# jameschapman19/cca_zoo

Measured on NVIDIA H100. Metric: rcca_fit_per_s, higher is better.
Workload: dtype tf32x3b+f32

## Files before the change

cca_zoo_b200/csrc/common.cuh:

```cuda
#pragma once

#include <cuda.h>
#include <cuda_runtime.h>
#include <stdint.h>
#include <stdio.h>

namespace ccab {

void set_error(const char* fmt, ...);
int cuda_fail(cudaError_t e, const char* what);

#define CCAB_CUDA(expr)                                              \
  do {                                                               \
    cudaError_t _e = (expr);                                         \
    if (_e != cudaSuccess) return ::ccab::cuda_fail(_e, #expr);      \
  } while (0)

#define CCAB_CHECK_ARG(cond, ...)        \
  do {                                   \
    if (!(cond)) {                       \
      ::ccab::set_error(__VA_ARGS__);    \
      return -1;                         \
    }                                    \
  } while (0)

void count_launches(int n);
long launch_count();

static inline int64_t ceil_div(int64_t a, int64_t b) { return (a + b - 1) / b; }

#ifdef __CUDACC__

__device__ __forceinline__ uint32_t smem_u32(const void* p) {
  return static_cast<uint32_t>(__cvta_generic_to_shared(p));
}

template <int N>
__device__ __forceinline__ void setmaxnreg_dec() { asm volatile("setmaxnreg.dec.sync.aligned.u32 %0;" ::"n"(N)); }
template <int N>
__device__ __forceinline__ void setmaxnreg_inc() { asm volatile("setmaxnreg.inc.sync.aligned.u32 %0;" ::"n"(N)); }

__device__ __forceinline__ void mbar_init(uint64_t* bar, uint32_t count) {
  asm volatile("mbarrier.init.shared::cta.b64 [%0], %1;" ::"r"(smem_u32(bar)), "r"(count) : "memory");
}
__device__ __forceinline__ void fence_mbar_init() {
  asm volatile("fence.mbarrier_init.release.cluster;" ::: "memory");
}
__device__ __forceinline__ void mbar_arrive(uint64_t* bar) {
  asm volatile("mbarrier.arrive.shared::cta.b64 _, [%0];" ::"r"(smem_u32(bar)) : "memory");
}
__device__ __forceinline__ void mbar_arrive_expect_tx(uint64_t* bar, uint32_t bytes) {
  asm volatile("mbarrier.arrive.expect_tx.shared::cta.b64 _, [%0], %1;" ::"r"(smem_u32(bar)), "r"(bytes)
               : "memory");
}
__device__ __forceinline__ bool mbar_try_wait(uint64_t* bar, uint32_t parity) {
  uint32_t ok;
  asm volatile(
      "{\n\t.reg .pred P1;\n\t"
      "mbarrier.try_wait.parity.shared::cta.b64 P1, [%1], %2;\n\t"
      "selp.b32 %0, 1, 0, P1;\n\t}\n"
      : "=r"(ok)
      : "r"(smem_u32(bar)), "r"(parity)
      : "memory");
  return ok != 0;
}
__device__ __forceinline__ void mbar_wait(uint64_t* bar, uint32_t parity) {
  uint32_t spins = 0;
  while (!mbar_try_wait(bar, parity)) {
    if (++spins > (1u << 25)) __trap();
  }
}

__device__ __forceinline__ void tma_load_2d(void* smem_dst, const CUtensorMap* map, uint64_t* bar, int c0, int c1) {
  asm volatile(
      "cp.async.bulk.tensor.2d.shared::cluster.global.mbarrier::complete_tx::bytes [%0], [%1, {%3, %4}], [%2];"
      ::"r"(smem_u32(smem_dst)), "l"(map), "r"(smem_u32(bar)), "r"(c0), "r"(c1)
      : "memory");
}


__device__ __forceinline__ void fence_proxy_async_smem() {
  asm volatile("fence.proxy.async.shared::cta;" ::: "memory");
}
__device__ __forceinline__ void wgmma_fence() { asm volatile("wgmma.fence.sync.aligned;" ::: "memory"); }
__device__ __forceinline__ void wgmma_commit() { asm volatile("wgmma.commit_group.sync.aligned;" ::: "memory"); }
__device__ __forceinline__ void wgmma_wait_all() { asm volatile("wgmma.wait_group.sync.aligned 0;" ::: "memory"); }
__device__ __forceinline__ void wgmma_wait_1() { asm volatile("wgmma.wait_group.sync.aligned 1;" ::: "memory"); }
template <int N>
__device__ __forceinline__ void wgmma_wait() { asm volatile("wgmma.wait_group.sync.aligned %0;" ::"n"(N) : "memory"); }
template <int R>
__device__ __forceinline__ void wgmma_fence_regs(float* d) {
#pragma unroll
  for (int i = 0; i < R; ++i) asm volatile("" : "+f"(d[i])::"memory");
}
template <int R>
__device__ __forceinline__ void wgmma_fence_regs(uint32_t* a) {
#pragma unroll
  for (int i = 0; i < R; ++i) asm volatile("" : "+r"(a[i])::"memory");
}

__device__ __forceinline__ uint64_t wgmma_desc_k128(uint32_t saddr) {
  return (uint64_t)((saddr >> 4) & 0x3FFF) | ((uint64_t)1 << 16) | ((uint64_t)(1024 >> 4) << 32) |
         ((uint64_t)1 << 62);
}

template <int N>
__device__ __forceinline__ void wgmma_tf32(float* d, uint64_t desc_a, uint64_t desc_b);

template <>
__device__ __forceinline__ void wgmma_tf32<64>(float* d, uint64_t desc_a, uint64_t desc_b) {
  asm volatile(
      "{\n\t.reg .pred p;\n\tsetp.ne.b32 p, %34, 0;\n\t"
      "wgmma.mma_async.sync.aligned.m64n64k8.f32.tf32.tf32 "
      "{%0, %1, %2, %3, %4, %5, %6, %7, %8, %9, %10, %11, %12, %13, %14, %15, %16, %17, %18, %19, %20, %21, %22, %23, %24, %25, %26, %27, %28, %29, %30, %31}, %32, %33, p, 1, 1;\n\t}\n"
      : "+f"(d[0]), "+f"(d[1]), "+f"(d[2]), "+f"(d[3]), "+f"(d[4]), "+f"(d[5]), "+f"(d[6]), "+f"(d[7]), "+f"(d[8]), "+f"(d[9]), "+f"(d[10]), "+f"(d[11]), "+f"(d[12]), "+f"(d[13]), "+f"(d[14]), "+f"(d[15]), "+f"(d[16]), "+f"(d[17]), "+f"(d[18]), "+f"(d[19]), "+f"(d[20]), "+f"(d[21]), "+f"(d[22]), "+f"(d[23]), "+f"(d[24]), "+f"(d[25]), "+f"(d[26]), "+f"(d[27]), "+f"(d[28]), "+f"(d[29]), "+f"(d[30]), "+f"(d[31])
      : "l"(desc_a), "l"(desc_b), "r"(1));
}

template <>
__device__ __forceinline__ void wgmma_tf32<128>(float* d, uint64_t desc_a, uint64_t desc_b) {
  asm volatile(
      "{\n\t.reg .pred p;\n\tsetp.ne.b32 p, %66, 0;\n\t"
      "wgmma.mma_async.sync.aligned.m64n128k8.f32.tf32.tf32 "
      "{%0, %1, %2, %3, %4, %5, %6, %7, %8, %9, %10, %11, %12, %13, %14, %15, %16, %17, %18, %19, %20, %21, %22, %23, %24, %25, %26, %27, %28, %29, %30, %31, %32, %33, %34, %35, %36, %37, %38, %39, %40, %41, %42, %43, %44, %45, %46, %47, %48, %49, %50, %51, %52, %53, %54, %55, %56, %57, %58, %59, %60, %61, %62, %63}, %64, %65, p, 1, 1;\n\t}\n"
      : "+f"(d[0]), "+f"(d[1]), "+f"(d[2]), "+f"(d[3]), "+f"(d[4]), "+f"(d[5]), "+f"(d[6]), "+f"(d[7]), "+f"(d[8]), "+f"(d[9]), "+f"(d[10]), "+f"(d[11]), "+f"(d[12]), "+f"(d[13]), "+f"(d[14]), "+f"(d[15]), "+f"(d[16]), "+f"(d[17]), "+f"(d[18]), "+f"(d[19]), "+f"(d[20]), "+f"(d[21]), "+f"(d[22]), "+f"(d[23]), "+f"(d[24]), "+f"(d[25]), "+f"(d[26]), "+f"(d[27]), "+f"(d[28]), "+f"(d[29]), "+f"(d[30]), "+f"(d[31]), "+f"(d[32]), "+f"(d[33]), "+f"(d[34]), "+f"(d[35]), "+f"(d[36]), "+f"(d[37]), "+f"(d[38]), "+f"(d[39]), "+f"(d[40]), "+f"(d[41]), "+f"(d[42]), "+f"(d[43]), "+f"(d[44]), "+f"(d[45]), "+f"(d[46]), "+f"(d[47]), "+f"(d[48]), "+f"(d[49]), "+f"(d[50]), "+f"(d[51]), "+f"(d[52]), "+f"(d[53]), "+f"(d[54]), "+f"(d[55]), "+f"(d[56]), "+f"(d[57]), "+f"(d[58]), "+f"(d[59]), "+f"(d[60]), "+f"(d[61]), "+f"(d[62]), "+f"(d[63])
      : "l"(desc_a), "l"(desc_b), "r"(1));
}

template <int N>
__device__ __forceinline__ void wgmma_tf32_ra(float* d, const uint32_t* a, uint64_t desc_b);

template <>
__device__ __forceinline__ void wgmma_tf32_ra<128>(float* d, const uint32_t* a, uint64_t desc_b) {
  asm volatile(
      "{\n\t.reg .pred p;\n\tsetp.ne.b32 p, %69, 0;\n\t"
      "wgmma.mma_async.sync.aligned.m64n128k8.f32.tf32.tf32 "
      "{%0, %1, %2, %3, %4, %5, %6, %7, %8, %9, %10, %11, %12, %13, %14, %15, %16, %17, %18, %19, %20, %21, %22, %23, %24, %25, %26, %27, %28, %29, %30, %31, %32, %33, %34, %35, %36, %37, %38, %39, %40, %41, %42, %43, %44, %45, %46, %47, %48, %49, %50, %51, %52, %53, %54, %55, %56, %57, %58, %59, %60, %61, %62, %63}, {%64, %65, %66, %67}, %68, p, 1, 1;\n\t}\n"
      : "+f"(d[0]), "+f"(d[1]), "+f"(d[2]), "+f"(d[3]), "+f"(d[4]), "+f"(d[5]), "+f"(d[6]), "+f"(d[7]), "+f"(d[8]), "+f"(d[9]), "+f"(d[10]), "+f"(d[11]), "+f"(d[12]), "+f"(d[13]), "+f"(d[14]), "+f"(d[15]), "+f"(d[16]), "+f"(d[17]), "+f"(d[18]), "+f"(d[19]), "+f"(d[20]), "+f"(d[21]), "+f"(d[22]), "+f"(d[23]), "+f"(d[24]), "+f"(d[25]), "+f"(d[26]), "+f"(d[27]), "+f"(d[28]), "+f"(d[29]), "+f"(d[30]), "+f"(d[31]), "+f"(d[32]), "+f"(d[33]), "+f"(d[34]), "+f"(d[35]), "+f"(d[36]), "+f"(d[37]), "+f"(d[38]), "+f"(d[39]), "+f"(d[40]), "+f"(d[41]), "+f"(d[42]), "+f"(d[43]), "+f"(d[44]), "+f"(d[45]), "+f"(d[46]), "+f"(d[47]), "+f"(d[48]), "+f"(d[49]), "+f"(d[50]), "+f"(d[51]), "+f"(d[52]), "+f"(d[53]), "+f"(d[54]), "+f"(d[55]), "+f"(d[56]), "+f"(d[57]), "+f"(d[58]), "+f"(d[59]), "+f"(d[60]), "+f"(d[61]), "+f"(d[62]), "+f"(d[63])
      : "r"(a[0]), "r"(a[1]), "r"(a[2]), "r"(a[3]), "l"(desc_b), "r"(1));
}

__device__ __forceinline__ float tf32_hi(float v) { return __uint_as_float(__float_as_uint(v) & 0xFFFFE000u); }
__device__ __forceinline__ float tf32_residual(float v) {
  uint32_t l;
  asm("cvt.rna.tf32.f32 %0, %1;" : "=r"(l) : "f"(v - tf32_hi(v)));
  return __uint_as_float(l);
}

__device__ __forceinline__ uint32_t k128_offset(int row, int kg) {
  return (uint32_t)row * 128u + ((uint32_t)(kg ^ (row & 7)) << 4);
}

template <bool KMAJ, int ROWS>
struct TileStager {
  static constexpr int kItems = ROWS * 8 / 256;
  float v[kItems][4];

  __device__ __forceinline__ static int item_row(int i) { return KMAJ ? i >> 3 : i % ROWS; }
  __device__ __forceinline__ static int item_kg(int i) { return KMAJ ? i & 7 : i / ROWS; }

  __device__ __forceinline__ void load(const float* X, int64_t ld, int rows, int ks, bool vec) {
#pragma unroll
    for (int j = 0; j < kItems; ++j) {
      const int i = threadIdx.x + 256 * j;
      const int r = item_row(i), k = 4 * item_kg(i);
      if (KMAJ) {
        const float* src = X + (int64_t)r * ld + k;
        if (vec && r < rows && k + 4 <= ks) {
          const float4 q = __ldg(reinterpret_cast<const float4*>(src));
          v[j][0] = q.x; v[j][1] = q.y; v[j][2] = q.z; v[j][3] = q.w;
        } else {
#pragma unroll
          for (int e = 0; e < 4; ++e) v[j][e] = (r < rows && k + e < ks) ? __ldg(src + e) : 0.f;
        }
      } else {
#pragma unroll
        for (int e = 0; e < 4; ++e) v[j][e] = (r < rows && k + e < ks) ? __ldg(X + (int64_t)(k + e) * ld + r) : 0.f;
      }
    }
  }

  template <bool X3>
  __device__ __forceinline__ void store(uint8_t* hi, uint8_t* lo) const {
#pragma unroll
    for (int j = 0; j < kItems; ++j) {
      const int i = threadIdx.x + 256 * j;
      const uint32_t off = k128_offset(item_row(i), item_kg(i));
      *reinterpret_cast<float4*>(hi + off) =
          make_float4(tf32_hi(v[j][0]), tf32_hi(v[j][1]), tf32_hi(v[j][2]), tf32_hi(v[j][3]));
      if (X3)
        *reinterpret_cast<float4*>(lo + off) = make_float4(tf32_residual(v[j][0]), tf32_residual(v[j][1]),
                                                           tf32_residual(v[j][2]), tf32_residual(v[j][3]));
    }
  }
};

#endif

}
```

cca_zoo_b200/csrc/moments.cu:

```cuda
#include "moments.cuh"

#include <mutex>
#include <type_traits>

namespace ccab {

int make_layout(int n_views, const int64_t* dims, ColumnLayout* L) {
  CCAB_CHECK_ARG(n_views >= 1 && n_views <= kMaxViews, "n_views must be in [1,%d], got %d", kMaxViews,
                 n_views);
  L->n_views = n_views;
  L->coff[0] = 0;
  L->poff[0] = 0;
  int nb = 0;
  for (int v = 0; v < n_views; ++v) {
    CCAB_CHECK_ARG(dims[v] >= 1 && dims[v] <= kMaxBlocks * kBlk, "bad view width %lld", (long long)dims[v]);
    L->dims[v] = (int)dims[v];
    int b = (int)ceil_div(dims[v], kBlk);
    nb += b;
    L->coff[v + 1] = L->coff[v] + (int)dims[v];
    L->poff[v + 1] = L->poff[v] + b * kBlk;
  }
  CCAB_CHECK_ARG(nb <= kMaxBlocks, "total padded width %d exceeds %d", nb * kBlk, kMaxBlocks * kBlk);
  L->nblocks = nb;
  L->D = L->coff[n_views];
  L->Dp = nb * kBlk;
  return 0;
}

static bool g_prof_on = false;
static cudaEvent_t g_prof_e0 = nullptr, g_prof_e1 = nullptr;
static bool g_prof_valid = false;
void moments_profile_enable(int on) {
  g_prof_on = on != 0;
  g_prof_valid = false;
  if (g_prof_on && !g_prof_e0) {
    cudaEventCreate(&g_prof_e0);
    cudaEventCreate(&g_prof_e1);
  }
}
float moments_profile_last_ms() {
  if (!g_prof_valid) return -1.f;
  float ms = -1.f;
  if (cudaEventSynchronize(g_prof_e1) != cudaSuccess) return -1.f;
  if (cudaEventElapsedTime(&ms, g_prof_e0, g_prof_e1) != cudaSuccess) return -1.f;
  return ms;
}

struct WgParams {
  CUtensorMap map[kMaxViews];
  uint8_t blk_view[kMaxBlocks];
  int blk_col0[kMaxBlocks];
  float* partial;
  float* partial_sum;
  int64_t n_rows, rows_per_split;
  int64_t row_base;
  int nblocks, Dp;
};
static_assert(sizeof(WgParams) <= 4096, "kernel parameter space");

constexpr int kWgXpose = 256;
constexpr int kWgThreads = kWgXpose + 256;
constexpr int kWgKC = 32;
constexpr int kWgTile = kBlk * kWgKC * 4;
constexpr int kWgBox = 32 * kWgKC * 4;

__device__ __forceinline__ uint32_t raw_offset(int k, int m) {
  return (uint32_t)(m >> 5) * kWgBox + k128_offset(k, (m & 31) >> 2) + (uint32_t)(m & 3) * 4;
}

template <bool X3>
struct WgCfg {
  static constexpr int kOps = X3 ? 2 : 1;
  static constexpr int kOpStage = kOps * kWgTile;
  static constexpr int kRawStage = 2 * kWgTile;
  static constexpr int kOpStages = X3 ? 2 : 3;
  static constexpr int kRawStages = 5;
  static constexpr int kBarOff = kOpStages * kOpStage + kRawStages * kRawStage;
  static constexpr int kSumOff = kBarOff + 2 * (kOpStages + kRawStages) * 8;
  static constexpr int kSmem = kSumOff + kBlk * 4 + 1024;
};
static_assert(WgCfg<true>::kSmem <= 227 * 1024 && WgCfg<false>::kSmem <= 227 * 1024, "shared memory per block");
static_assert(WgCfg<true>::kRawStages > WgCfg<true>::kOpStages && WgCfg<false>::kRawStages > WgCfg<false>::kOpStages,
              "the refill of a raw stage must not wait on the MMA warps' current slice");

template <bool X3>
__global__ void __launch_bounds__(kWgThreads, 1) moments_wgmma_kernel(const __grid_constant__ WgParams p) {
  using Cfg = WgCfg<X3>;
  constexpr int NO = Cfg::kOpStages, NR = Cfg::kRawStages;
  extern __shared__ uint8_t smem_raw[];
  uint8_t* smem = smem_raw + ((1024u - (smem_u32(smem_raw) & 1023u)) & 1023u);
  uint8_t* ops = smem;
  uint8_t* raw = smem + NO * Cfg::kOpStage;
  uint64_t* raw_full = reinterpret_cast<uint64_t*>(smem + Cfg::kBarOff);
  uint64_t* raw_empty = raw_full + NR;
  uint64_t* op_full = raw_empty + NR;
  uint64_t* op_empty = op_full + NO;

  int t = blockIdx.x, bi = 0, rowlen = p.nblocks;
  while (t >= rowlen) { t -= rowlen; ++bi; --rowlen; }
  const int bj = bi + t;
  const bool diag = bi == bj;
  const int split = blockIdx.y;
  const int64_t r0 = (int64_t)split * p.rows_per_split;
  const int64_t r1 = min(r0 + p.rows_per_split, p.n_rows);
  const int nch = r1 > r0 ? (int)((r1 - r0 + kWgKC - 1) / kWgKC) : 0;

  if (threadIdx.x == 0) {
    for (int s = 0; s < NR; ++s) {
      mbar_init(&raw_full[s], 1);
      mbar_init(&raw_empty[s], kWgXpose + 8);
    }
    for (int s = 0; s < NO; ++s) {
      mbar_init(&op_full[s], kWgXpose);
      mbar_init(&op_empty[s], 8);
    }
    fence_mbar_init();
  }
  __syncthreads();

  if (threadIdx.x < kWgXpose) {
    setmaxnreg_dec<80>();
    const int m = threadIdx.x % kBlk, h = threadIdx.x / kBlk;
    const CUtensorMap* mapA = &p.map[p.blk_view[bi]];
    const CUtensorMap* mapB = &p.map[p.blk_view[bj]];
    const int colA = p.blk_col0[bi], colB = p.blk_col0[bj];
    auto issue = [&](int c) {
      const int s = c % NR;
      const int row = (int)(p.row_base + r0 + (int64_t)c * kWgKC);
      uint8_t* dst = raw + s * Cfg::kRawStage;
      mbar_arrive_expect_tx(&raw_full[s], diag ? kWgTile : 2 * kWgTile);
#pragma unroll
      for (int q = 0; q < kBlk / 32; ++q) {
        tma_load_2d(dst + q * kWgBox, mapA, &raw_full[s], colA + 32 * q, row);
        if (!diag) tma_load_2d(dst + kWgTile + q * kWgBox, mapB, &raw_full[s], colB + 32 * q, row);
      }
    };
    if (threadIdx.x == 0)
      for (int c = 0; c < min(NR, nch); ++c) issue(c);

    float csum = 0.f;
    auto transpose = [&](const uint8_t* src, uint8_t* hi, uint8_t* lo, bool sums) {
#pragma unroll
      for (int j = 0; j < kWgKC / 8; ++j) {
        const int kg = 2 * j + h;
        float v[4];
#pragma unroll
        for (int e = 0; e < 4; ++e)
          v[e] = *reinterpret_cast<const float*>(src + raw_offset(4 * kg + e, m));
        const uint32_t off = k128_offset(m, kg);
        *reinterpret_cast<float4*>(hi + off) = make_float4(tf32_hi(v[0]), tf32_hi(v[1]), tf32_hi(v[2]), tf32_hi(v[3]));
        if (X3)
          *reinterpret_cast<float4*>(lo + off) = make_float4(tf32_residual(v[0]), tf32_residual(v[1]),
                                                             tf32_residual(v[2]), tf32_residual(v[3]));
        if (sums) csum += (v[0] + v[1]) + (v[2] + v[3]);
      }
    };
    for (int c = 0; c < nch; ++c) {
      const int sr = c % NR, so = c % NO;
      mbar_wait(&raw_full[sr], (c / NR) & 1);
      mbar_wait(&op_empty[so], ((c / NO) & 1) ^ 1);
      uint8_t* dst = ops + so * Cfg::kOpStage;
      transpose(raw + sr * Cfg::kRawStage + (diag ? 0 : kWgTile), dst, dst + kWgTile, diag);
      fence_proxy_async_smem();
      mbar_arrive(&raw_empty[sr]);
      mbar_arrive(&op_full[so]);
      const int rf = c + NR - NO + 1;
      if (threadIdx.x == 0 && rf >= NR && rf < nch) {
        mbar_wait(&raw_empty[rf % NR], (rf / NR - 1) & 1);
        issue(rf);
      }
    }
    if (diag) {
      float* odd = reinterpret_cast<float*>(smem + Cfg::kSumOff);
      if (h) odd[m] = csum;
      asm volatile("bar.sync 1, %0;" ::"n"(kWgXpose) : "memory");
      if (!h) p.partial_sum[(size_t)split * p.Dp + bi * kBlk + m] = csum + odd[m];
    }
  } else {
    setmaxnreg_inc<168>();
    const int wg = (threadIdx.x - kWgXpose) >> 7, lane = threadIdx.x & 31, t = lane & 3;
    const int m = wg * 64 + ((threadIdx.x >> 5) & 3) * 16 + (lane >> 2);
    const int kx = t ^ ((t & 1) << 2);
    const bool swap = t & 1;
    const uint32_t o00 = raw_offset(kx, m), o01 = raw_offset(kx ^ 4, m);
    const uint32_t o10 = raw_offset(kx, m + 8), o11 = raw_offset(kx ^ 4, m + 8);
    float acc[64];
#pragma unroll
    for (int i = 0; i < 64; ++i) acc[i] = 0.f;
    wgmma_fence_regs<64>(acc);
    constexpr int KS = kWgKC / 8;
    uint32_t fa[KS][Cfg::kOps][4] = {};
    for (int c = 0; c < nch; ++c) {
      const int sr = c % NR, so = c % NO;
      mbar_wait(&raw_full[sr], (c / NR) & 1);
      const uint8_t* a_src = raw + sr * Cfg::kRawStage;
      const uint32_t b0 = smem_u32(ops + so * Cfg::kOpStage);
#pragma unroll
      for (int kk = 0; kk < KS; ++kk) {
        wgmma_wait<KS - 1>();
        wgmma_fence_regs<Cfg::kOps * 4>(&fa[kk][0][0]);
        if (kk == KS - 1 && c > 0 && lane == 0) mbar_arrive(&op_empty[(c - 1) % NO]);
        const uint8_t* s = a_src + kk * 1024;
        const float v00 = *reinterpret_cast<const float*>(s + o00), v01 = *reinterpret_cast<const float*>(s + o01);
        const float v10 = *reinterpret_cast<const float*>(s + o10), v11 = *reinterpret_cast<const float*>(s + o11);
        const float a[4] = {swap ? v01 : v00, swap ? v11 : v10, swap ? v00 : v01, swap ? v10 : v11};
#pragma unroll
        for (int i = 0; i < 4; ++i) {
          fa[kk][0][i] = __float_as_uint(tf32_hi(a[i]));
          if constexpr (X3) fa[kk][1][i] = __float_as_uint(tf32_residual(a[i]));
        }
        wgmma_fence_regs<Cfg::kOps * 4>(&fa[kk][0][0]);
        if (kk == KS - 1) {
          __syncwarp();
          if (lane == 0) mbar_arrive(&raw_empty[sr]);
        }
        if (kk == 0) mbar_wait(&op_full[so], (c / NO) & 1);
        const uint64_t b_hi = wgmma_desc_k128(b0 + 32 * kk);
        wgmma_fence();
        if constexpr (X3) {
          const uint64_t b_lo = wgmma_desc_k128(b0 + kWgTile + 32 * kk);
          wgmma_tf32_ra<128>(acc, fa[kk][1], b_hi);
          wgmma_tf32_ra<128>(acc, fa[kk][0], b_lo);
        }
        wgmma_tf32_ra<128>(acc, fa[kk][0], b_hi);
        wgmma_commit();
      }
    }
    wgmma_wait_all();
    wgmma_fence_regs<64>(acc);

    const int warp = (threadIdx.x >> 5) & 3;
    float* P = p.partial + (size_t)split * p.Dp * p.Dp;
    const int row0 = bi * kBlk + wg * 64 + warp * 16 + (lane >> 2);
    const int col0 = bj * kBlk + 2 * (lane & 3);
#pragma unroll
    for (int r = 0; r < 64; r += 2) {
      const int row = row0 + 8 * ((r >> 1) & 1), col = col0 + 8 * (r >> 2);
      *reinterpret_cast<float2*>(P + (size_t)row * p.Dp + col) = make_float2(acc[r], acc[r + 1]);
    }
  }
}
struct SimtParams {
  const void* view_ptr[kMaxViews];
  int64_t view_ld[kMaxViews];
  int view_dim[kMaxViews];
  int view_poff[kMaxViews + 1];
  int n_views;
  int64_t n_rows;
  int64_t rows_per_split;
  int nb64, Dp;
  void* partial;
  void* partial_sum;
};

template <typename T>
__global__ void __launch_bounds__(256) moments_simt_kernel(const SimtParams p) {
  constexpr int KC = 16;
  __shared__ T As[KC][64];
  __shared__ T Bs[KC][64];
  int t = blockIdx.x, bi = 0, rowlen = p.nb64;
  while (t >= rowlen) { t -= rowlen; ++bi; --rowlen; }
  const int bj = bi + t;
  const int split = blockIdx.y;
  const int64_t r0 = split * p.rows_per_split;
  const int64_t r1 = min(r0 + p.rows_per_split, p.n_rows);

  auto locate = [&](int pcol0, int& v, int& c0) {
    v = 0;
    while (v + 1 < p.n_views && p.view_poff[v + 1] <= pcol0) ++v;
    c0 = pcol0 - p.view_poff[v];
  };
  int vA, cA, vB, cB;
  locate(bi * 64, vA, cA);
  locate(bj * 64, vB, cB);
  const T* XA = static_cast<const T*>(p.view_ptr[vA]);
  const T* XB = static_cast<const T*>(p.view_ptr[vB]);
  const int64_t ldA = p.view_ld[vA], ldB = p.view_ld[vB];
  const int dA = p.view_dim[vA], dB = p.view_dim[vB];

  const int tx = threadIdx.x & 15, ty = threadIdx.x >> 4;
  T acc[4][4];
#pragma unroll
  for (int i = 0; i < 4; ++i)
#pragma unroll
    for (int j = 0; j < 4; ++j) acc[i][j] = T(0);
  T csum[4] = {T(0), T(0), T(0), T(0)};
  constexpr int kRun = 2048;
  double fold[4][4], fold_sum[4];
#pragma unroll
  for (int i = 0; i < 4; ++i) {
    fold_sum[i] = 0.0;
#pragma unroll
    for (int j = 0; j < 4; ++j) fold[i][j] = 0.0;
  }
  auto fold_run = [&]() {
#pragma unroll
    for (int i = 0; i < 4; ++i) {
      fold_sum[i] += (double)csum[i];
      csum[i] = T(0);
#pragma unroll
      for (int j = 0; j < 4; ++j) {
        fold[i][j] += (double)acc[i][j];
        acc[i][j] = T(0);
      }
    }
  };

  const int lc = threadIdx.x & 63, lr = threadIdx.x >> 6;
  for (int64_t r = r0; r < r1; r += KC) {
    if (r > r0 && (r - r0) % kRun == 0) fold_run();
#pragma unroll
    for (int i = 0; i < KC / 4; ++i) {
      const int kr = lr + 4 * i;
      const int64_t row = r + kr;
      const bool rv = row < r1;
      As[kr][lc] = (rv && cA + lc < dA) ? XA[row * ldA + cA + lc] : T(0);
      Bs[kr][lc] = (rv && cB + lc < dB) ? XB[row * ldB + cB + lc] : T(0);
    }
    __syncthreads();
#pragma unroll
    for (int k = 0; k < KC; ++k) {
      T a[4], b[4];
#pragma unroll
      for (int i = 0; i < 4; ++i) { a[i] = As[k][ty * 4 + i]; b[i] = Bs[k][tx * 4 + i]; }
#pragma unroll
      for (int i = 0; i < 4; ++i)
#pragma unroll
        for (int j = 0; j < 4; ++j) acc[i][j] = fma(a[i], b[j], acc[i][j]);
      if (ty == 0) {
#pragma unroll
        for (int j = 0; j < 4; ++j) csum[j] += b[j];
      }
    }
    __syncthreads();
  }
  fold_run();
  T* P = static_cast<T*>(p.partial) + (size_t)split * p.Dp * p.Dp;
#pragma unroll
  for (int i = 0; i < 4; ++i)
#pragma unroll
    for (int j = 0; j < 4; ++j)
      P[(size_t)(bi * 64 + ty * 4 + i) * p.Dp + bj * 64 + tx * 4 + j] = (T)fold[i][j];
  if (bi == bj && ty == 0) {
    T* S = static_cast<T*>(p.partial_sum) + (size_t)split * p.Dp;
#pragma unroll
    for (int j = 0; j < 4; ++j) S[bi * 64 + tx * 4 + j] = (T)fold_sum[j];
  }
}

__device__ __forceinline__ void dmma_m8n8k4(double& c0, double& c1, double a, double b) {
  asm volatile("mma.sync.aligned.m8n8k4.row.col.f64.f64.f64.f64 {%0, %1}, {%2}, {%3}, {%0, %1};"
               : "+d"(c0), "+d"(c1)
               : "d"(a), "d"(b));
}

__global__ void __launch_bounds__(256) moments_dmma_kernel(const SimtParams p) {
  constexpr int KC = 16;
  constexpr int LDS = 64 + 4;
  __shared__ double As[2][KC][LDS];
  __shared__ double Bs[2][KC][LDS];
  int t = blockIdx.x, bi = 0, rowlen = p.nb64;
  while (t >= rowlen) { t -= rowlen; ++bi; --rowlen; }
  const int bj = bi + t;
  const int split = blockIdx.y;
  const int64_t r0 = split * p.rows_per_split;
  const int64_t r1 = min(r0 + p.rows_per_split, p.n_rows);

  auto locate = [&](int pcol0, int& v, int& c0) {
    v = 0;
    while (v + 1 < p.n_views && p.view_poff[v + 1] <= pcol0) ++v;
    c0 = pcol0 - p.view_poff[v];
  };
  int vA, cA, vB, cB;
  locate(bi * 64, vA, cA);
  locate(bj * 64, vB, cB);
  const double* XA = static_cast<const double*>(p.view_ptr[vA]);
  const double* XB = static_cast<const double*>(p.view_ptr[vB]);
// ... 142 lines not shown
}

struct TcPlan {
  int total_chunks, num_splits, chunks_per_split, ntiles;
  size_t partial_bytes, sum_bytes;
};

TcPlan plan_tc(const ColumnLayout& L, int64_t n_rows, int mode) {
  const bool x3 = mode != 0;
  TcPlan P;
  P.total_chunks = (int)ceil_div(n_rows, kWgKC);
  P.ntiles = L.nblocks * (L.nblocks + 1) / 2;
  int S = (int)ceil_div(4 * sm_count(), P.ntiles);
  int max_splits = 64;
  if (x3) {
    S = std::max<int64_t>(S, ceil_div(n_rows, 2048));
    max_splits = 256;
  }
  const int min_chunks = 8;
  S = (int)std::min<int64_t>(S, std::max<int64_t>(1, P.total_chunks / min_chunks));
  const int64_t slab = (int64_t)L.Dp * L.Dp * (int64_t)sizeof(float);
  max_splits = (int)std::max<int64_t>(1, std::min<int64_t>(max_splits, ((int64_t)2 << 30) / slab));
  S = std::min(S, max_splits);
  S = std::max(1, std::min(S, P.total_chunks));
  P.chunks_per_split = (int)ceil_div(P.total_chunks, S);
  P.num_splits = (int)ceil_div(P.total_chunks, P.chunks_per_split);
  P.partial_bytes = (size_t)P.num_splits * L.Dp * L.Dp * sizeof(float);
  P.sum_bytes = (size_t)P.num_splits * L.Dp * sizeof(float);
  return P;
}

int64_t tc_rows_cap(const ColumnLayout& L, int mode) {
  if (mode == 0) return (int64_t)1 << 31;
  const int64_t slab = (int64_t)L.Dp * L.Dp * (int64_t)sizeof(float);
  const int64_t max_splits = std::max<int64_t>(1, std::min<int64_t>(256, ((int64_t)2 << 30) / slab));
  return max_splits * 2048;
}

inline size_t align256(size_t x) { return (x + 255) & ~size_t(255); }

struct SimtPlan {
  int nb64, ntiles, num_splits;
  int64_t rows_per_split;
};

SimtPlan plan_simt(const ColumnLayout& L, int64_t n_rows) {
  SimtPlan P;
  P.nb64 = L.Dp / 64;
  P.ntiles = P.nb64 * (P.nb64 + 1) / 2;
  int S = 1;
  if (P.ntiles < 2 * sm_count()) S = (2 * sm_count()) / P.ntiles;
  S = (int)std::min<int64_t>(S, std::max<int64_t>(1, n_rows / 64));
  S = std::max(1, std::min(S, 64));
  P.rows_per_split = ceil_div(ceil_div(n_rows, S), 16) * 16;
  P.num_splits = (int)ceil_div(n_rows, P.rows_per_split);
  return P;
}

}

size_t moments_workspace_bytes(int dtype, int precision, const ColumnLayout& L, int64_t n_rows) {
  if (precision == 2 || dtype == 1) {
    SimtPlan P = plan_simt(L, n_rows);
    size_t el = dtype == 1 ? 8 : 4;
    return align256((size_t)P.num_splits * L.Dp * L.Dp * el) + align256((size_t)P.num_splits * L.Dp * el);
  }
  TcPlan P = plan_tc(L, std::min(n_rows, tc_rows_cap(L, precision)), precision);
  return align256(P.partial_bytes) + align256(P.sum_bytes) + 256;
}

namespace {

typedef CUresult (*EncodeTiledFn)(CUtensorMap*, CUtensorMapDataType, cuuint32_t, void*, const cuuint64_t*,
                                  const cuuint64_t*, const cuuint32_t*, const cuuint32_t*, CUtensorMapInterleave,
                                  CUtensorMapSwizzle, CUtensorMapL2promotion, CUtensorMapFloatOOBfill);

EncodeTiledFn encode_fn() {
  static EncodeTiledFn fn = nullptr;
  static std::once_flag once;
  std::call_once(once, [] {
    void* f = nullptr;
    cudaDriverEntryPointQueryResult q;
    if (cudaGetDriverEntryPoint("cuTensorMapEncodeTiled", &f, cudaEnableDefault, &q) == cudaSuccess &&
        q == cudaDriverEntryPointSuccess)
      fn = reinterpret_cast<EncodeTiledFn>(f);
  });
  return fn;
}

int encode_view_map(CUtensorMap* map, const void* ptr, int64_t n_rows, int64_t d, int64_t ld) {
  EncodeTiledFn enc = encode_fn();
  if (!enc) {
    set_error("cuTensorMapEncodeTiled entry point not available (driver too old?)");
    return -2;
  }
  cuuint64_t gdim[2] = {(cuuint64_t)d, (cuuint64_t)n_rows};
  cuuint64_t gstride[1] = {(cuuint64_t)ld * 4};
  cuuint32_t box[2] = {32, (cuuint32_t)kWgKC};
  cuuint32_t estr[2] = {1, 1};
  CUresult r = enc(map, CU_TENSOR_MAP_DATA_TYPE_FLOAT32, 2, const_cast<void*>(ptr), gdim, gstride, box, estr,
                   CU_TENSOR_MAP_INTERLEAVE_NONE, CU_TENSOR_MAP_SWIZZLE_128B, CU_TENSOR_MAP_L2_PROMOTION_L2_256B,
                   CU_TENSOR_MAP_FLOAT_OOB_FILL_NONE);
  if (r != CUDA_SUCCESS) {
    set_error("cuTensorMapEncodeTiled failed with CUresult %d (d=%lld n=%lld ld=%lld)", (int)r, (long long)d,
              (long long)n_rows, (long long)ld);
    return -3;
  }
  return 0;
}

int moments_tf32_pass(const ColumnLayout& L, WgParams& prm, int64_t row_base, int64_t n_rows, int mode,
                      double* moments_out, void* ws, size_t ws_bytes, cudaStream_t stream, int accumulate);

}

int moments_tf32(const ColumnLayout& L, const void* const* views, const int64_t* lds, int64_t n_rows, int mode,
                 double* moments_out, void* ws, size_t ws_bytes, cudaStream_t stream) {
  CCAB_CHECK_ARG(n_rows >= 1 && n_rows < (int64_t)1 << 31, "n_rows out of range");
  for (int v = 0; v < L.n_views; ++v)
    CCAB_CHECK_ARG((reinterpret_cast<uintptr_t>(views[v]) & 15) == 0 && lds[v] % 4 == 0,
                   "TF32 moments need 16-byte aligned views and lds %% 4 == 0 (view %d: ld %lld)", v,
                   (long long)lds[v]);
  {
    int dev = 0;
    CCAB_CUDA(cudaGetDevice(&dev));
    CCAB_CUDA(cudaSetDevice(dev));
  }
  WgParams prm;
  memset(&prm, 0, sizeof(prm));
  for (int v = 0; v < L.n_views; ++v) {
    int rc = encode_view_map(&prm.map[v], views[v], n_rows, L.dims[v], lds[v]);
    if (rc) return rc;
  }
  int b = 0;
  for (int v = 0; v < L.n_views; ++v)
    for (int c = 0; c < L.dims[v]; c += kBlk, ++b) {
      prm.blk_view[b] = (uint8_t)v;
      prm.blk_col0[b] = c;
    }
  const int64_t cap = tc_rows_cap(L, mode);
  if (n_rows <= cap) return moments_tf32_pass(L, prm, 0, n_rows, mode, moments_out, ws, ws_bytes, stream, 0);
  const int64_t npass = ceil_div(n_rows, cap);
  const int64_t per = std::min(cap, ceil_div(ceil_div(n_rows, npass), 2048) * 2048);
  int pass = 0;
  for (int64_t r0 = 0; r0 < n_rows; r0 += per, ++pass) {
    int rc = moments_tf32_pass(L, prm, r0, std::min(per, n_rows - r0), mode, moments_out, ws, ws_bytes, stream,
                               pass > 0);
    if (rc) return rc;
  }
  return 0;
}

namespace {
int moments_tf32_pass(const ColumnLayout& L, WgParams& prm, int64_t row_base, int64_t n_rows, int mode,
                      double* moments_out, void* ws, size_t ws_bytes, cudaStream_t stream, int accumulate) {
  TcPlan P = plan_tc(L, n_rows, mode);
  const size_t need = align256(P.partial_bytes) + align256(P.sum_bytes) + 256;
  CCAB_CHECK_ARG(ws_bytes >= need, "workspace too small: %zu < %zu", ws_bytes, need);
  uint8_t* w = reinterpret_cast<uint8_t*>((reinterpret_cast<uintptr_t>(ws) + 255) & ~uintptr_t(255));
  float* d_partial = reinterpret_cast<float*>(w);
  float* d_partial_sum = reinterpret_cast<float*>(w + align256(P.partial_bytes));

  prm.partial = d_partial;
  prm.partial_sum = d_partial_sum;
  prm.n_rows = n_rows;
  prm.rows_per_split = (int64_t)P.chunks_per_split * kWgKC;
  prm.row_base = row_base;
  prm.nblocks = L.nblocks;
  prm.Dp = L.Dp;
  dim3 grid(P.ntiles, P.num_splits);
  if (g_prof_on) cudaEventRecord(g_prof_e0, stream);
  if (mode != 0) {
    CCAB_CUDA(cudaFuncSetAttribute(moments_wgmma_kernel<true>, cudaFuncAttributeMaxDynamicSharedMemorySize,
                                   WgCfg<true>::kSmem));
    moments_wgmma_kernel<true><<<grid, kWgThreads, WgCfg<true>::kSmem, stream>>>(prm);
  } else {
    CCAB_CUDA(cudaFuncSetAttribute(moments_wgmma_kernel<false>, cudaFuncAttributeMaxDynamicSharedMemorySize,
                                   WgCfg<false>::kSmem));
    moments_wgmma_kernel<false><<<grid, kWgThreads, WgCfg<false>::kSmem, stream>>>(prm);
  }
  count_launches(1);
  CCAB_CUDA(cudaGetLastError());
  if (g_prof_on) {
    cudaEventRecord(g_prof_e1, stream);
    g_prof_valid = true;
  }

  const size_t total = (size_t)L.Dp * L.Dp + L.Dp;
  int rblocks = (int)std::min<size_t>((total + 255) / 256, (size_t)sm_count() * 8);
  reduce_partials_kernel<float><<<rblocks, 256, 0, stream>>>(d_partial, d_partial_sum, P.num_splits, L.Dp, L.Dp,
                                                            kBlk, moments_out, accumulate); count_launches(1);
  CCAB_CUDA(cudaGetLastError());
  return 0;
}
}

template <typename T>
int moments_simt(const ColumnLayout& L, const void* const* views, const int64_t* lds, int64_t n_rows,
                 double* moments_out, void* ws, size_t ws_bytes, cudaStream_t stream) {
  CCAB_CHECK_ARG(n_rows >= 1, "n_rows must be positive");
  SimtPlan P = plan_simt(L, n_rows);
  const size_t pb = align256((size_t)P.num_splits * L.Dp * L.Dp * sizeof(T));
  const size_t sb = align256((size_t)P.num_splits * L.Dp * sizeof(T));
  CCAB_CHECK_ARG(ws_bytes >= pb + sb, "workspace too small: %zu < %zu", ws_bytes, pb + sb);
  uint8_t* w = static_cast<uint8_t*>(ws);
  SimtParams prm;
  memset(&prm, 0, sizeof(prm));
  for (int v = 0; v < L.n_views; ++v) {
    prm.view_ptr[v] = views[v];
    prm.view_ld[v] = lds[v];
    prm.view_dim[v] = L.dims[v];
  }
  for (int v = 0; v <= L.n_views; ++v) prm.view_poff[v] = L.poff[v];
  prm.n_views = L.n_views;
  prm.n_rows = n_rows;
  prm.rows_per_split = P.rows_per_split;
  prm.nb64 = P.nb64;
  prm.Dp = L.Dp;
  prm.partial = w;
  prm.partial_sum = w + pb;
  dim3 grid(P.ntiles, P.num_splits);
  if constexpr (std::is_same<T, double>::value)
    moments_dmma_kernel<<<grid, 256, 0, stream>>>(prm);
  else
    moments_simt_kernel<T><<<grid, 256, 0, stream>>>(prm);
  count_launches(1);
  CCAB_CUDA(cudaGetLastError());
  const size_t total = (size_t)L.Dp * L.Dp + L.Dp;
  int rblocks = (int)std::min<size_t>((total + 255) / 256, (size_t)sm_count() * 8);
  reduce_partials_kernel<T><<<rblocks, 256, 0, stream>>>(static_cast<const T*>(prm.partial),
                                                        static_cast<const T*>(prm.partial_sum), P.num_splits,
                                                        L.Dp, L.Dp, 64, moments_out); count_launches(1);
  CCAB_CUDA(cudaGetLastError());
  return 0;
}

template int moments_simt<float>(const ColumnLayout&, const void* const*, const int64_t*, int64_t, double*, void*,
                                 size_t, cudaStream_t);
template int moments_simt<double>(const ColumnLayout&, const void* const*, const int64_t*, int64_t, double*, void*,
                                  size_t, cudaStream_t);

__global__ void pack_moments_kernel(const double* __restrict__ mom, int nblocks, int Dp, double n_local,
                                    double* __restrict__ packed) {
  const int nt = nblocks * (nblocks + 1) / 2;
  const int t = blockIdx.x;
  if (t < nt) {
    int bi = 0, rem = t, rowlen = nblocks;
    while (rem >= rowlen) { rem -= rowlen; ++bi; --rowlen; }
    const int bj = bi + rem;
    const double* src = mom + (size_t)bi * kBlk * Dp + (size_t)bj * kBlk;
    double* dst = packed + (size_t)t * kBlk * kBlk;
    for (int e = threadIdx.x; e < kBlk * kBlk; e += blockDim.x) dst[e] = src[(size_t)(e / kBlk) * Dp + (e % kBlk)];
  } else {
    double* dst = packed + (size_t)nt * kBlk * kBlk;
    const double* s = mom + (size_t)Dp * Dp;
    for (int e = threadIdx.x; e < Dp; e += blockDim.x) dst[e] = s[e];
    if (threadIdx.x == 0) { dst[Dp] = n_local; dst[Dp + 1] = 0.0; }
  }
}

__global__ void unpack_moments_kernel(const double* __restrict__ packed, int nblocks, int Dp, double* __restrict__ mom) {
  const int nt = nblocks * (nblocks + 1) / 2;
  const int bi = blockIdx.y, bj = blockIdx.x;
  if (bi < nblocks) {
    double* dst = mom + (size_t)bi * kBlk * Dp + (size_t)bj * kBlk;
    if (bj >= bi) {
      const int t = bi * nblocks - bi * (bi - 1) / 2 + (bj - bi);
      const double* src = packed + (size_t)t * kBlk * kBlk;
      for (int e = threadIdx.x; e < kBlk * kBlk; e += blockDim.x) dst[(size_t)(e / kBlk) * Dp + (e % kBlk)] = src[e];
    } else {
      for (int e = threadIdx.x; e < kBlk * kBlk; e += blockDim.x) dst[(size_t)(e / kBlk) * Dp + (e % kBlk)] = 0.0;
    }
  } else if (bj == 0) {
    const double* src = packed + (size_t)nt * kBlk * kBlk;
    double* s = mom + (size_t)Dp * Dp;
    for (int e = threadIdx.x; e < Dp; e += blockDim.x) s[e] = src[e];
  }
}

__device__ __forceinline__ double multimem_ld_reduce_add_f64(const double* mc_addr) {
  double v;
  asm volatile("multimem.ld_reduce.relaxed.sys.global.add.f64 %0, [%1];" : "=d"(v) : "l"(mc_addr) : "memory");
  return v;
}
__device__ __forceinline__ void multimem_st_f64(double* mc_addr, double v) {
  asm volatile("multimem.st.relaxed.sys.global.f64 [%0], %1;" ::"l"(mc_addr), "d"(v) : "memory");
}
__device__ __forceinline__ void st_release_sys_u32(uint32_t* p, uint32_t v) {
  asm volatile("st.release.sys.global.u32 [%0], %1;" ::"l"(p), "r"(v) : "memory");
}
__device__ __forceinline__ uint32_t ld_acquire_sys_u32(const uint32_t* p) {
  uint32_t v;
  asm volatile("ld.acquire.sys.global.u32 %0, [%1];" : "=r"(v) : "l"(p) : "memory");
  return v;
}

struct ExchangeParams {
  double* mom;
  double* sym;
  double* mc;
  uint32_t* const* pads;
  double* n_total_out;
  double n_local;
  long long packed;
  long long chunk;
  int rank, world, nblocks, Dp;
  unsigned epoch;
};

__device__ __forceinline__ const double* packed_src(const ExchangeParams& p, long long e, int nt) {
  const long long blk = e / (kBlk * kBlk);
  if (blk < nt) {
    int bi = 0, rem = (int)blk, rowlen = p.nblocks;
    while (rem >= rowlen) { rem -= rowlen; ++bi; --rowlen; }
    const int bj = bi + rem;
    const int off = (int)(e - blk * (kBlk * kBlk));
    return p.mom + ((size_t)bi * kBlk + off / kBlk) * p.Dp + (size_t)bj * kBlk + (off % kBlk);
  }
  const long long t = e - (long long)nt * kBlk * kBlk;
  return t < p.Dp ? p.mom + (size_t)p.Dp * p.Dp + t : nullptr;
}

__device__ __forceinline__ void exchange_barrier(const ExchangeParams& p, unsigned value) {
  __threadfence_system();
  __syncthreads();
  if ((int)threadIdx.x < p.world)
    st_release_sys_u32(p.pads[threadIdx.x] + (size_t)blockIdx.x * p.world + p.rank, value);
  if ((int)threadIdx.x < p.world) {
    const uint32_t* slot = p.pads[p.rank] + (size_t)blockIdx.x * p.world + threadIdx.x;
    unsigned spins = 0;
    while ((int)(ld_acquire_sys_u32(slot) - value) < 0) {
      if (++spins > (1u << 26)) {
        printf("ccab: exchange barrier timed out (rank %d cta %d peer %d)\n", p.rank, blockIdx.x, threadIdx.x);
// ... 228 lines not shown
```

Measured before the change: 147.0.

## Add X3B mode computing cross terms of 3xTF32 with BF16 wgmma

Adds a third kernel mode in which the hi×lo and lo×hi correction products of the split-precision moment GEMM run as BF16 m64n128k16 wgmma instead of TF32 k8. The hi parts stay TF32. The transpose stage writes BF16-packed hi and residual operands alongside the TF32 hi tile. The aim is to halve the instruction count of the correction terms and use the faster BF16 tensor-core rate. In exchange the correction terms carry less precision, and the change only takes effect when mode 3 is selected.

New measurement: 162.7 (median of 6 runs). +10.7%, better.

```diff
diff --git a/cca_zoo_b200/csrc/common.cuh b/cca_zoo_b200/csrc/common.cuh
--- a/cca_zoo_b200/csrc/common.cuh
+++ b/cca_zoo_b200/csrc/common.cuh
@@ -138,6 +138,25 @@
       "{%0, %1, %2, %3, %4, %5, %6, %7, %8, %9, %10, %11, %12, %13, %14, %15, %16, %17, %18, %19, %20, %21, %22, %23, %24, %25, %26, %27, %28, %29, %30, %31, %32, %33, %34, %35, %36, %37, %38, %39, %40, %41, %42, %43, %44, %45, %46, %47, %48, %49, %50, %51, %52, %53, %54, %55, %56, %57, %58, %59, %60, %61, %62, %63}, {%64, %65, %66, %67}, %68, p, 1, 1;\n\t}\n"
       : "+f"(d[0]), "+f"(d[1]), "+f"(d[2]), "+f"(d[3]), "+f"(d[4]), "+f"(d[5]), "+f"(d[6]), "+f"(d[7]), "+f"(d[8]), "+f"(d[9]), "+f"(d[10]), "+f"(d[11]), "+f"(d[12]), "+f"(d[13]), "+f"(d[14]), "+f"(d[15]), "+f"(d[16]), "+f"(d[17]), "+f"(d[18]), "+f"(d[19]), "+f"(d[20]), "+f"(d[21]), "+f"(d[22]), "+f"(d[23]), "+f"(d[24]), "+f"(d[25]), "+f"(d[26]), "+f"(d[27]), "+f"(d[28]), "+f"(d[29]), "+f"(d[30]), "+f"(d[31]), "+f"(d[32]), "+f"(d[33]), "+f"(d[34]), "+f"(d[35]), "+f"(d[36]), "+f"(d[37]), "+f"(d[38]), "+f"(d[39]), "+f"(d[40]), "+f"(d[41]), "+f"(d[42]), "+f"(d[43]), "+f"(d[44]), "+f"(d[45]), "+f"(d[46]), "+f"(d[47]), "+f"(d[48]), "+f"(d[49]), "+f"(d[50]), "+f"(d[51]), "+f"(d[52]), "+f"(d[53]), "+f"(d[54]), "+f"(d[55]), "+f"(d[56]), "+f"(d[57]), "+f"(d[58]), "+f"(d[59]), "+f"(d[60]), "+f"(d[61]), "+f"(d[62]), "+f"(d[63])
       : "r"(a[0]), "r"(a[1]), "r"(a[2]), "r"(a[3]), "l"(desc_b), "r"(1));
+}
+
+template <int N>
+__device__ __forceinline__ void wgmma_bf16_ra(float* d, const uint32_t* a, uint64_t desc_b);
+
+template <>
+__device__ __forceinline__ void wgmma_bf16_ra<128>(float* d, const uint32_t* a, uint64_t desc_b) {
+  asm volatile(
+      "{\n\t.reg .pred p;\n\tsetp.ne.b32 p, %69, 0;\n\t"
+      "wgmma.mma_async.sync.aligned.m64n128k16.f32.bf16.bf16 "
+      "{%0, %1, %2, %3, %4, %5, %6, %7, %8, %9, %10, %11, %12, %13, %14, %15, %16, %17, %18, %19, %20, %21, %22, %23, %24, %25, %26, %27, %28, %29, %30, %31, %32, %33, %34, %35, %36, %37, %38, %39, %40, %41, %42, %43, %44, %45, %46, %47, %48, %49, %50, %51, %52, %53, %54, %55, %56, %57, %58, %59, %60, %61, %62, %63}, {%64, %65, %66, %67}, %68, p, 1, 1, 0;\n\t}\n"
+      : "+f"(d[0]), "+f"(d[1]), "+f"(d[2]), "+f"(d[3]), "+f"(d[4]), "+f"(d[5]), "+f"(d[6]), "+f"(d[7]), "+f"(d[8]), "+f"(d[9]), "+f"(d[10]), "+f"(d[11]), "+f"(d[12]), "+f"(d[13]), "+f"(d[14]), "+f"(d[15]), "+f"(d[16]), "+f"(d[17]), "+f"(d[18]), "+f"(d[19]), "+f"(d[20]), "+f"(d[21]), "+f"(d[22]), "+f"(d[23]), "+f"(d[24]), "+f"(d[25]), "+f"(d[26]), "+f"(d[27]), "+f"(d[28]), "+f"(d[29]), "+f"(d[30]), "+f"(d[31]), "+f"(d[32]), "+f"(d[33]), "+f"(d[34]), "+f"(d[35]), "+f"(d[36]), "+f"(d[37]), "+f"(d[38]), "+f"(d[39]), "+f"(d[40]), "+f"(d[41]), "+f"(d[42]), "+f"(d[43]), "+f"(d[44]), "+f"(d[45]), "+f"(d[46]), "+f"(d[47]), "+f"(d[48]), "+f"(d[49]), "+f"(d[50]), "+f"(d[51]), "+f"(d[52]), "+f"(d[53]), "+f"(d[54]), "+f"(d[55]), "+f"(d[56]), "+f"(d[57]), "+f"(d[58]), "+f"(d[59]), "+f"(d[60]), "+f"(d[61]), "+f"(d[62]), "+f"(d[63])
+      : "r"(a[0]), "r"(a[1]), "r"(a[2]), "r"(a[3]), "l"(desc_b), "r"(1));
+}
+
+__device__ __forceinline__ uint32_t pack_bf16x2(float lo, float hi) {
+  uint32_t r;
+  asm("cvt.rn.bf16x2.f32 %0, %1, %2;" : "=r"(r) : "f"(hi), "f"(lo));
+  return r;
 }
 
 __device__ __forceinline__ float tf32_hi(float v) { return __uint_as_float(__float_as_uint(v) & 0xFFFFE000u); }
diff --git a/cca_zoo_b200/csrc/moments.cu b/cca_zoo_b200/csrc/moments.cu
--- a/cca_zoo_b200/csrc/moments.cu
+++ b/cca_zoo_b200/csrc/moments.cu
@@ -68,24 +68,30 @@
   return (uint32_t)(m >> 5) * kWgBox + k128_offset(k, (m & 31) >> 2) + (uint32_t)(m & 3) * 4;
 }
 
-template <bool X3>
+enum class K1Mode { TF32, X3, X3B };
+
+template <K1Mode M>
 struct WgCfg {
-  static constexpr int kOps = X3 ? 2 : 1;
+  static constexpr int kOps = M == K1Mode::TF32 ? 1 : 2;
   static constexpr int kOpStage = kOps * kWgTile;
   static constexpr int kRawStage = 2 * kWgTile;
-  static constexpr int kOpStages = X3 ? 2 : 3;
+  static constexpr int kOpStages = M == K1Mode::TF32 ? 3 : 2;
   static constexpr int kRawStages = 5;
   static constexpr int kBarOff = kOpStages * kOpStage + kRawStages * kRawStage;
   static constexpr int kSumOff = kBarOff + 2 * (kOpStages + kRawStages) * 8;
   static constexpr int kSmem = kSumOff + kBlk * 4 + 1024;
 };
-static_assert(WgCfg<true>::kSmem <= 227 * 1024 && WgCfg<false>::kSmem <= 227 * 1024, "shared memory per block");
-static_assert(WgCfg<true>::kRawStages > WgCfg<true>::kOpStages && WgCfg<false>::kRawStages > WgCfg<false>::kOpStages,
+static_assert(WgCfg<K1Mode::X3>::kSmem <= 227 * 1024 && WgCfg<K1Mode::TF32>::kSmem <= 227 * 1024 &&
+              WgCfg<K1Mode::X3B>::kSmem <= 227 * 1024, "shared memory per block");
+static_assert(WgCfg<K1Mode::X3>::kRawStages > WgCfg<K1Mode::X3>::kOpStages &&
+              WgCfg<K1Mode::TF32>::kRawStages > WgCfg<K1Mode::TF32>::kOpStages &&
+              WgCfg<K1Mode::X3B>::kRawStages > WgCfg<K1Mode::X3B>::kOpStages,
               "the refill of a raw stage must not wait on the MMA warps' current slice");
 
-template <bool X3>
+template <K1Mode M>
 __global__ void __launch_bounds__(kWgThreads, 1) moments_wgmma_kernel(const __grid_constant__ WgParams p) {
-  using Cfg = WgCfg<X3>;
+  using Cfg = WgCfg<M>;
+  constexpr bool X3 = M == K1Mode::X3;
   constexpr int NO = Cfg::kOpStages, NR = Cfg::kRawStages;
   extern __shared__ uint8_t smem_raw[];
   uint8_t* smem = smem_raw + ((1024u - (smem_u32(smem_raw) & 1023u)) & 1023u);
@@ -140,19 +146,41 @@
 
     float csum = 0.f;
     auto transpose = [&](const uint8_t* src, uint8_t* hi, uint8_t* lo, bool sums) {
-#pragma unroll
-      for (int j = 0; j < kWgKC / 8; ++j) {
-        const int kg = 2 * j + h;
-        float v[4];
-#pragma unroll
-        for (int e = 0; e < 4; ++e)
-          v[e] = *reinterpret_cast<const float*>(src + raw_offset(4 * kg + e, m));
-        const uint32_t off = k128_offset(m, kg);
-        *reinterpret_cast<float4*>(hi + off) = make_float4(tf32_hi(v[0]), tf32_hi(v[1]), tf32_hi(v[2]), tf32_hi(v[3]));
-        if (X3)
-          *reinterpret_cast<float4*>(lo + off) = make_float4(tf32_residual(v[0]), tf32_residual(v[1]),
-                                                             tf32_residual(v[2]), tf32_residual(v[3]));
-        if (sums) csum += (v[0] + v[1]) + (v[2] + v[3]);
+      if constexpr (M == K1Mode::X3B) {
+#pragma unroll
+        for (int q = 0; q < 2; ++q) {
+          const int e = 2 * h + q;
+          float v[8], x[8];
+#pragma unroll
+          for (int i = 0; i < 8; ++i) {
+            v[i] = *reinterpret_cast<const float*>(src + raw_offset(8 * e + i, m));
+            x[i] = tf32_hi(v[i]);
+          }
+          *reinterpret_cast<float4*>(hi + k128_offset(m, 2 * e)) = make_float4(x[0], x[1], x[2], x[3]);
+          *reinterpret_cast<float4*>(hi + k128_offset(m, 2 * e + 1)) = make_float4(x[4], x[5], x[6], x[7]);
+          *reinterpret_cast<uint4*>(lo + k128_offset(m, e)) =
+              make_uint4(pack_bf16x2(x[0], x[4]), pack_bf16x2(x[1], x[5]), pack_bf16x2(x[2], x[6]),
+                         pack_bf16x2(x[3], x[7]));
+          *reinterpret_cast<uint4*>(lo + k128_offset(m, 4 + e)) =
+              make_uint4(pack_bf16x2(v[0] - x[0], v[4] - x[4]), pack_bf16x2(v[1] - x[1], v[5] - x[5]),
+                         pack_bf16x2(v[2] - x[2], v[6] - x[6]), pack_bf16x2(v[3] - x[3], v[7] - x[7]));
+          if (sums) csum += ((v[0] + v[1]) + (v[2] + v[3])) + ((v[4] + v[5]) + (v[6] + v[7]));
+        }
+      } else {
+#pragma unroll
+        for (int j = 0; j < kWgKC / 8; ++j) {
+          const int kg = 2 * j + h;
+          float v[4];
+#pragma unroll
+          for (int e = 0; e < 4; ++e)
+            v[e] = *reinterpret_cast<const float*>(src + raw_offset(4 * kg + e, m));
+          const uint32_t off = k128_offset(m, kg);
+          *reinterpret_cast<float4*>(hi + off) = make_float4(tf32_hi(v[0]), tf32_hi(v[1]), tf32_hi(v[2]), tf32_hi(v[3]));
+          if (X3)
+            *reinterpret_cast<float4*>(lo + off) = make_float4(tf32_residual(v[0]), tf32_residual(v[1]),
+                                                               tf32_residual(v[2]), tf32_residual(v[3]));
+          if (sums) csum += (v[0] + v[1]) + (v[2] + v[3]);
+        }
       }
     };
     for (int c = 0; c < nch; ++c) {
@@ -188,8 +216,10 @@
 #pragma unroll
     for (int i = 0; i < 64; ++i) acc[i] = 0.f;
     wgmma_fence_regs<64>(acc);
-    constexpr int KS = kWgKC / 8;
-    uint32_t fa[KS][Cfg::kOps][4] = {};
+    constexpr int KQ = M == K1Mode::X3B ? 2 : 1;
+    constexpr int KS = kWgKC / (8 * KQ);
+    constexpr int KR = M == K1Mode::X3B ? 16 : Cfg::kOps * 4;
+    uint32_t fa[KS][KR] = {};
     for (int c = 0; c < nch; ++c) {
       const int sr = c % NR, so = c % NO;
       mbar_wait(&raw_full[sr], (c / NR) & 1);
@@ -198,31 +228,50 @@
 #pragma unroll
       for (int kk = 0; kk < KS; ++kk) {
         wgmma_wait<KS - 1>();
-        wgmma_fence_regs<Cfg::kOps * 4>(&fa[kk][0][0]);
+        wgmma_fence_regs<KR>(fa[kk]);
         if (kk == KS - 1 && c > 0 && lane == 0) mbar_arrive(&op_empty[(c - 1) % NO]);
-        const uint8_t* s = a_src + kk * 1024;
-        const float v00 = *reinterpret_cast<const float*>(s + o00), v01 = *reinterpret_cast<const float*>(s + o01);
-        const float v10 = *reinterpret_cast<const float*>(s + o10), v11 = *reinterpret_cast<const float*>(s + o11);
-        const float a[4] = {swap ? v01 : v00, swap ? v11 : v10, swap ? v00 : v01, swap ? v10 : v11};
-#pragma unroll
-        for (int i = 0; i < 4; ++i) {
-          fa[kk][0][i] = __float_as_uint(tf32_hi(a[i]));
-          if constexpr (X3) fa[kk][1][i] = __float_as_uint(tf32_residual(a[i]));
+#pragma unroll
+        for (int q = 0; q < KQ; ++q) {
+          const uint8_t* s = a_src + (KQ * kk + q) * 1024;
+          const float v00 = *reinterpret_cast<const float*>(s + o00), v01 = *reinterpret_cast<const float*>(s + o01);
+          const float v10 = *reinterpret_cast<const float*>(s + o10), v11 = *reinterpret_cast<const float*>(s + o11);
+          const float a[4] = {swap ? v01 : v00, swap ? v11 : v10, swap ? v00 : v01, swap ? v10 : v11};
+          float x[4];
+#pragma unroll
+          for (int i = 0; i < 4; ++i) {
+            x[i] = tf32_hi(a[i]);
+            fa[kk][4 * q + i] = __float_as_uint(x[i]);
+            if constexpr (X3) fa[kk][4 + i] = __float_as_uint(tf32_residual(a[i]));
+          }
+          if constexpr (M == K1Mode::X3B) {
+#pragma unroll
+            for (int r = 0; r < 2; ++r) {
+              fa[kk][8 + 2 * q + r] = pack_bf16x2(x[r], x[r + 2]);
+              fa[kk][12 + 2 * q + r] = pack_bf16x2(a[r] - x[r], a[r + 2] - x[r + 2]);
+            }
+          }
         }
-        wgmma_fence_regs<Cfg::kOps * 4>(&fa[kk][0][0]);
+        wgmma_fence_regs<KR>(fa[kk]);
         if (kk == KS - 1) {
           __syncwarp();
           if (lane == 0) mbar_arrive(&raw_empty[sr]);
         }
         if (kk == 0) mbar_wait(&op_full[so], (c / NO) & 1);
-        const uint64_t b_hi = wgmma_desc_k128(b0 + 32 * kk);
         wgmma_fence();
-        if constexpr (X3) {
-          const uint64_t b_lo = wgmma_desc_k128(b0 + kWgTile + 32 * kk);
-          wgmma_tf32_ra<128>(acc, fa[kk][1], b_hi);
-          wgmma_tf32_ra<128>(acc, fa[kk][0], b_lo);
+        if constexpr (M == K1Mode::X3B) {
+          wgmma_bf16_ra<128>(acc, &fa[kk][12], wgmma_desc_k128(b0 + kWgTile + 32 * kk));
+          wgmma_bf16_ra<128>(acc, &fa[kk][8], wgmma_desc_k128(b0 + kWgTile + 64 + 32 * kk));
+          wgmma_tf32_ra<128>(acc, &fa[kk][0], wgmma_desc_k128(b0 + 64 * kk));
+          wgmma_tf32_ra<128>(acc, &fa[kk][4], wgmma_desc_k128(b0 + 64 * kk + 32));
+        } else {
+          const uint64_t b_hi = wgmma_desc_k128(b0 + 32 * kk);
+          if constexpr (X3) {
+            const uint64_t b_lo = wgmma_desc_k128(b0 + kWgTile + 32 * kk);
+            wgmma_tf32_ra<128>(acc, &fa[kk][4], b_hi);
+            wgmma_tf32_ra<128>(acc, &fa[kk][0], b_lo);
+          }
+          wgmma_tf32_ra<128>(acc, &fa[kk][0], b_hi);
         }
-        wgmma_tf32_ra<128>(acc, fa[kk][0], b_hi);
         wgmma_commit();
       }
     }
@@ -671,6 +720,14 @@
 }
 
 namespace {
+template <K1Mode M>
+int launch_wgmma(dim3 grid, const WgParams& prm, cudaStream_t stream) {
+  CCAB_CUDA(cudaFuncSetAttribute(moments_wgmma_kernel<M>, cudaFuncAttributeMaxDynamicSharedMemorySize,
+                                 WgCfg<M>::kSmem));
+  moments_wgmma_kernel<M><<<grid, kWgThreads, WgCfg<M>::kSmem, stream>>>(prm);
+  return 0;
+}
+
 int moments_tf32_pass(const ColumnLayout& L, WgParams& prm, int64_t row_base, int64_t n_rows, int mode,
                       double* moments_out, void* ws, size_t ws_bytes, cudaStream_t stream, int accumulate) {
   TcPlan P = plan_tc(L, n_rows, mode);
@@ -689,15 +746,10 @@
   prm.Dp = L.Dp;
   dim3 grid(P.ntiles, P.num_splits);
   if (g_prof_on) cudaEventRecord(g_prof_e0, stream);
-  if (mode != 0) {
-    CCAB_CUDA(cudaFuncSetAttribute(moments_wgmma_kernel<true>, cudaFuncAttributeMaxDynamicSharedMemorySize,
-                                   WgCfg<true>::kSmem));
-    moments_wgmma_kernel<true><<<grid, kWgThreads, WgCfg<true>::kSmem, stream>>>(prm);
-  } else {
-    CCAB_CUDA(cudaFuncSetAttribute(moments_wgmma_kernel<false>, cudaFuncAttributeMaxDynamicSharedMemorySize,
-                                   WgCfg<false>::kSmem));
-    moments_wgmma_kernel<false><<<grid, kWgThreads, WgCfg<false>::kSmem, stream>>>(prm);
-  }
+  int rc = mode == 3   ? launch_wgmma<K1Mode::X3B>(grid, prm, stream)
+           : mode != 0 ? launch_wgmma<K1Mode::X3>(grid, prm, stream)
+                       : launch_wgmma<K1Mode::TF32>(grid, prm, stream);
+  if (rc) return rc;
   count_launches(1);
   CCAB_CUDA(cudaGetLastError());
   if (g_prof_on) {
```
